# harmoniqs/DirectTrajOpt.jl

Hardware: AMD Instinct MI355X
Metric: knot-points/sec for eval_constraint_jacobian, 256-state×2000-knot bilinear (higher is better)
Workload: dtype f64; 1 GPU; configs[2]: 256-state bilinear, 4 drives, N=2000 knots per GPU (make_scaled_problem shape, Philox seed 42), callback=jacobian; state_dim=256, drives=4, knots_per_gpu=2000, knots_total=2000, parallelism=knot-range shards x1, outputs_finite=True, max_squarings=1, sweep_terms=25

## Files before the change

### directtrajopt.jl_amd/csrc/dto_engine.cpp

```cpp
#include "dto_handle.h"
#include "dto_rollout_plan.h"

#include <chrono>
#include <cmath>
#include <cstddef>
#include <cstdlib>
#include <cstring>
#include <initializer_list>
#include <limits>
#include <map>

using namespace dto;

thread_local std::string dto::g_create_error;

dto_handle::~dto_handle() {
    if (structure_only) return;
    (void)hipSetDevice(device);
    comm.reset();
    for (auto& r : prof) {
        (void)hipEventDestroy(r.a);
        (void)hipEventDestroy(r.b);
    }
    for (auto& e : ev_pool) (void)hipEventDestroy(e);
    for (void* p : owned) (void)hipFree(p);
    if (mailbox) (void)hipHostFree(mailbox);
    if (stream) (void)hipStreamDestroy(stream);
    if (stream2) (void)hipStreamDestroy(stream2);
    if (stream_rb) (void)hipStreamDestroy(stream_rb);
    if (ev_rb) (void)hipEventDestroy(ev_rb);
    if (ev_fork) (void)hipEventDestroy(ev_fork);
    if (ev_zero) (void)hipEventDestroy(ev_zero);
    if (ev_join) (void)hipEventDestroy(ev_join);
    if (ev_stats) (void)hipEventDestroy(ev_stats);
    if (ev_chain) (void)hipEventDestroy(ev_chain);
    if (ev_done) (void)hipEventDestroy(ev_done);
    if (h_stats) (void)hipHostFree(h_stats);
}

namespace {

struct ProfScope {
    dto_handle* h;
    hipStream_t st;
    bool on;
    ProfRec r{};
    ProfScope(dto_handle* h_, hipStream_t st_, int cat, double flops) : h(h_), st(st_), on(h_->profiling) {
        if (!on) return;
        r.cat = cat;
        r.flops = flops;
        auto take = [&](hipEvent_t& e) {
            if (h->ev_pool.empty()) (void)hipEventCreate(&e);
            else { e = h->ev_pool.back(); h->ev_pool.pop_back(); }
        };
        take(r.a);
        take(r.b);
        (void)hipEventRecord(r.a, st);
    }
    ~ProfScope() {
        if (!on) return;
        (void)hipEventRecord(r.b, st);
        h->prof.push_back(r);
    }
};
enum { CAT_BGEMM = 0, CAT_SWEEP = 1, CAT_OTHER = 2, CAT_BGEMM_HORNER = 3, CAT_BGEMM_SQUARE = 4, CAT_SWEEP_ADJOINT = 5,
       CAT_ZERO = 6, CAT_BUILD_A = 7, CAT_ASSEMBLY = 8, CAT_BASIS_MULTI = 9, CAT_CHAIN64 = 10, CAT_HESS_PRODUCT = 11, CAT_SHARE = 12, CAT_TDB_MFMA = 13, CAT_JAC_PRODUCT = 14, CAT_TDB_KRON = 15, CAT_TDB_PRODUCT = 16, CAT_ROLLOUT = 17, CAT_ROLLOUT_TREE = 18, CAT_ROLLOUT_DESCENT = 19, CAT_DYNSOLVE_TREE = 20, CAT_DYNSOLVE_SCAN = 21 };
inline bool is_rollout_cat(int cat) { return cat >= CAT_ROLLOUT && cat <= CAT_ROLLOUT_DESCENT; }
inline bool is_dynsolve_cat(int cat) { return cat == CAT_DYNSOLVE_TREE || cat == CAT_DYNSOLVE_SCAN; }
inline void count_sweep_form(dto_handle* h, int form) {
    if (h->profiling) ++h->sweep_forms[form];
}

}


namespace dto {

ShardExtents shard_extents(const dto_handle* h, int64_t k_lo, int64_t k_hi) {
    const int64_t kn_lo = k_lo - 1, n_knots = k_hi - k_lo + 1;
    const int64_t c_lo = kn_lo * h->z, c_hi = (kn_lo + n_knots) * h->z;
    const bool last = k_hi == h->N;
    ShardExtents e;
    e.grad_lo = c_lo;
    e.grad_len = c_hi - c_lo + (last ? h->gd : 0);
    e.jac_lo = h->colptr[c_lo];
    e.jac_len = h->colptr[last ? h->n_vars : c_hi] - e.jac_lo;
    e.hess_lo = hess_block_start(slab_dims(h), kn_lo);
    e.hess_len = hess_block_start(slab_dims(h), kn_lo + n_knots) - e.hess_lo + (last ? (int64_t)h->tail_rows.size() : 0);
    return e;
}

std::vector<std::pair<int64_t, int64_t>> shard_row_segments(const dto_handle* h, int64_t k_lo, int64_t k_hi) {
    const int64_t kn_lo = k_lo - 1, n_knots = k_hi - k_lo + 1;
    const int64_t n_int = std::max<int64_t>(0, std::min<int64_t>(k_hi, h->K) - k_lo + 1);
    std::vector<std::pair<int64_t, int64_t>> seg;
    for (size_t i = 0; i < h->integ_kind.size(); ++i)
        if (n_int > 0) seg.emplace_back(h->integ_row_off[i] + kn_lo * h->integ_dim[i], n_int * h->integ_dim[i]);
    for (auto& c : h->con) {
        int64_t prev = -2;
        for (int64_t i = 0; i < c.n_times_total; ++i) {
            const int64_t kn = c.times0[i];
            if (kn >= h->N ? k_hi != h->N : (kn < kn_lo || kn >= kn_lo + n_knots)) continue;
            if (!seg.empty() && prev == i - 1 && seg.back().first + seg.back().second == c.row_off + i * c.g_dim)
                seg.back().second += c.g_dim;
            else
                seg.emplace_back(c.row_off + i * c.g_dim, c.g_dim);
            prev = i;
        }
    }
    return seg;
}

}

namespace {



struct Bounds {
    double beta, b1;
};
Bounds read_bounds(const dto_handle* h) { return Bounds{h->mailbox->bounds[0], h->mailbox->bounds[1]}; }

void enqueue_bounds(dto_handle* h, BilHost& b, const double* dZ, hipStream_t st) {
    HIP_CHECK(hipMemsetAsync(h->d_bounds, 0, 2 * sizeof(double), st));
    launch_norm_bounds(st, h->P, b.k, dZ, b.d_g1, b.d_n2, reinterpret_cast<unsigned long long*>(h->d_bounds));
    HIP_CHECK(hipMemcpyAsync(h->mailbox->bounds, h->d_bounds, 2 * sizeof(double), hipMemcpyDeviceToHost, st));
}
Bounds get_bounds(dto_handle* h, BilHost& b, const double* dZ, hipStream_t st) {
    enqueue_bounds(h, b, dZ, st);
    HIP_CHECK(hipStreamSynchronize(st));
    return read_bounds(h);
}
// ... 109 lines not shown
                ps.r.flops += flops_step;
                if (a.store) {
                    ws.Z[0] = w.Zt + (size_t)t * tstride;
                    ws.Z[1] = w.Zt + (size_t)(t + 1) * tstride;
                    const bool split = ty.T == 1 && (int64_t)(t + b.k.m + 4) <= (int64_t)w.dcap * (1 + b.k.m);
                    launch_sweep_step(st, b.k, ws, ty, a.transposed, t, 0, split ? 1 : 0);
                } else {
                    launch_sweep_step(st, b.k, w, ty, a.transposed, t, buf);
                }
            }
            if (t >= tc) launch_sweep_check(st, w, ty.T, t, 1.1e-16);
            buf ^= 1;
            launched = t + 1;
            if (t >= 3 && (t % 4) == 3 && t + 1 < plan.d_ub) {
                int32_t* hs = h->mailbox->sweep_stats;
                if (pending) {
                    HIP_CHECK(hipEventSynchronize(h->ev_stats));
                    if (hs[slot ^ 1] == 0) break;
                }
                HIP_CHECK(hipMemcpyAsync(hs + slot, w.stats, sizeof(int32_t), hipMemcpyDeviceToHost, st));
                HIP_CHECK(hipEventRecord(h->ev_stats, st));
                pending = true;
                slot ^= 1;
            }
        }
    }
    return launched;
}

struct ChainChunks {
    int cap = 0;
    std::function<void(int64_t, int)> done;
};

struct ChainCall {
    ChainChunks chunks;
    std::function<void()> in_bubble;
    std::function<void(double)> after_last_enqueue;
    bool nothing_waits = false;
};

void run_chain(dto_handle* h, BilHost& b, const double* dZ, double* vals, hipStream_t st, const ChainCall& call) {
    const int npad = b.k.npad;
    const int64_t nint = h->P.n_int;
    double d2max = 0.0;
    if (nint <= 0) return;
    int cap = h->chain_chunk > 0 ? std::min(h->chain_chunk, b.chain_cap) : b.chain_cap;
    if (call.chunks.cap > 0 && !h->deterministic) cap = std::min(cap, call.chunks.cap);
    const int s_ub = 60;
    if (chain64_applies(h, b)) {
        ChainWork& w = b.chain;
        HIP_CHECK(hipMemsetAsync(w.smax, 0, 8 * sizeof(int32_t), st));
        HIP_CHECK(hipMemsetAsync(b.d_hump, 0, 8 * sizeof(unsigned long long), st));
        const int want_form = h->expm_form == 2 || h->expm_form == 3 ? h->expm_form : 0;
        {
            ProfScope ps(h, st, CAT_CHAIN64, 6.0 * 2.0 * 64.0 * 64.0 * 64.0 * (double)nint);
            HIP_CHECK(launch_chain64(st, h->P, b.k, dZ, vals, w.norms, w.smax, w.d2max, w.s, s_ub, want_form, h->n_cu));
        }
        if (call.nothing_waits) {
            HIP_CHECK(hipMemcpyAsync(&h->mailbox->deferred_smax, w.smax, sizeof(int32_t), hipMemcpyDeviceToHost, st));
            h->smax_pending = true;
            h->last_form = 0;
            if (call.in_bubble) call.in_bubble();
            if (call.chunks.done) call.chunks.done(0, (int)nint);
            if (call.after_last_enqueue) call.after_last_enqueue(0.0);
            return;
        }
        launch_hump(st, h->P, b.k, dZ, b.d_g1, h->P.kn_lo, (int)nint, w.norms, b.d_hump);
        const ChainReadback& rb = h->mailbox->chain;
        HIP_CHECK(hipMemcpyAsync(&h->mailbox->chain, w.smax, sizeof(ChainReadback), hipMemcpyDeviceToHost, st));
        HIP_CHECK(hipMemcpyAsync(h->mailbox->hump, b.d_hump, 8 * sizeof(unsigned long long), hipMemcpyDeviceToHost, st));
        HIP_CHECK(hipEventRecord(h->ev_chain, st));
        if (call.in_bubble) call.in_bubble();
        HIP_CHECK(hipEventSynchronize(h->ev_chain));
        h->last_form = 0;
        h->last_smax = rb.s_max2;
        read_hump(h, b);
        d2max = rb.d2max;
        if (call.chunks.done) call.chunks.done(0, (int)nint);
        if (call.after_last_enqueue) call.after_last_enqueue(d2max);
        return;
    }
    const double gemm_flops = 2.0 * npad * (double)npad * npad;
    h->last_smax = 0;
    const int64_t nchunk = (nint + cap - 1) / cap;
    const int per = (int)std::min<int64_t>(cap, (((nint + nchunk - 1) / nchunk) + 7) / 8 * 8);
    for (int64_t c0 = 0; c0 < nint; c0 += per) {
        const int nb = (int)std::min<int64_t>(per, nint - c0);
        const int64_t int0 = h->P.kn_lo + c0;
        ChainWork& w = b.chain;
        const int nbpad = ((nb + 127) / 128) * 128;
        if (b.use_basis) {
            launch_fill(st, w.norms, (int64_t)nb * 4, INFINITY);
            double* outs[3] = {w.W[1], w.W[2], w.W[3]};
            const size_t cs_set = (size_t)cap * npad * (npad / 64);
            double* css[3] = {w.colsum, w.colsum + cs_set, w.colsum + 2 * cs_set};
            {
                ProfScope ps(h, st, CAT_BUILD_A, 8.0 * npad * (double)npad * nb);
                launch_build_A(st, h->P, b.k, dZ, int0, nb, w.W[0]);
            }
            launch_basis_coef_multi(st, h->P, b.k, 3, b.basis, dZ, int0, nb, nbpad);
            {
                const double cols = b.basis[0].cntpad + b.basis[1].cntpad + b.basis[2].cntpad;
                ProfScope ps(h, st, CAT_BASIS_MULTI, 2.0 * npad * (double)npad * cols * nb);
                launch_basis_gemm_multi(st, npad, nb, nbpad, 3, b.basis, outs, css);
            }
            launch_norm_from_colsum_multi(st, npad, nb, 3, css, w.norms);
        } else {
            {
                ProfScope ps(h, st, CAT_BUILD_A, 8.0 * npad * (double)npad * nb);
                launch_build_A(st, h->P, b.k, dZ, int0, nb, w.W[0]);
            }
            { ProfScope ps(h, st, CAT_BGEMM, gemm_flops * nb); launch_bgemm_plain(st, npad, nb, w.W[0], w.W[0], w.W[1]); }
            { ProfScope ps(h, st, CAT_BGEMM, gemm_flops * nb); launch_bgemm_plain(st, npad, nb, w.W[0], w.W[1], w.W[2]); }
            { ProfScope ps(h, st, CAT_BGEMM, gemm_flops * nb); launch_bgemm_plain(st, npad, nb, w.W[1], w.W[1], w.W[3]); }
            launch_norm1(st, npad, nb, w);
        }
        HIP_CHECK(hipMemsetAsync(w.smax, 0, 8 * sizeof(int32_t), st));
        launch_expm_params(st, nb, s_ub, w);
        if (c0 == 0) HIP_CHECK(hipMemsetAsync(b.d_hump, 0, 8 * sizeof(unsigned long long), st));
        launch_hump(st, h->P, b.k, dZ, b.d_g1, int0, nb, w.norms, b.d_hump);
        launch_expm_coef(st, nb, w, h->expm_form == 2 || h->expm_form == 3 ? h->expm_form : 0);
        const ChainReadback& rb = h->mailbox->chain;
        HIP_CHECK(hipEventRecord(h->ev_rb, st));
        HIP_CHECK(hipStreamWaitEvent(h->stream_rb, h->ev_rb, 0));
        HIP_CHECK(hipMemcpyAsync(&h->mailbox->chain, w.smax, sizeof(ChainReadback), hipMemcpyDeviceToHost, h->stream_rb));
        HIP_CHECK(hipMemcpyAsync(h->mailbox->hump, b.d_hump, 8 * sizeof(unsigned long long), hipMemcpyDeviceToHost, h->stream_rb));
        HIP_CHECK(hipEventRecord(h->ev_chain, h->stream_rb));
        if (b.use_basis) {
            launch_basis_coef(st, h->P, b.k, b.basis_all, dZ, int0, nb, nbpad, w.coef);
            ProfScope ps(h, st, CAT_OTHER, 2.0 * npad * (double)npad * b.basis_all.cntpad * nb);
            launch_basis_gemm(st, npad, nb, nbpad, b.basis_all, w.W[5], nullptr);
        } else {
            launch_poly_h3(st, npad, nb, w);
        }
        if (c0 == 0 && call.in_bubble) call.in_bubble();
        HIP_CHECK(hipEventSynchronize(h->ev_chain));
        const int form = rb.form;
        if (form != 2 && form != 3) throw HipError{"propagator chain: the evaluation form did not come back from the device"};
        h->last_form = form;
        { ProfScope ps(h, st, CAT_BGEMM_HORNER, gemm_flops * nb); launch_bgemm_poly(st, npad, nb, w, 3, 5, 4, COEF_PA, 6, COEF_PB); }
        const SlabDest slab{h->P, b.k, int0, vals};
        if (form == 2) {
            ProfScope ps(h, st, CAT_BGEMM_HORNER, gemm_flops * nb);
            launch_bgemm_poly(st, npad, nb, w, 4, 6, 5, COEF_PC, -1, 0, false, &slab);
        } else {
            { ProfScope ps(h, st, CAT_BGEMM_HORNER, gemm_flops * nb); launch_bgemm_poly(st, npad, nb, w, 4, 6, 7, COEF_L, 8, COEF_R, true); }
            { ProfScope ps(h, st, CAT_BGEMM_HORNER, gemm_flops * nb); launch_bgemm_poly(st, npad, nb, w, 7, 8, 5, COEF_PC, -1, 0, false, &slab); }
        }
        const int s_max = form == 3 ? rb.s_max3 : rb.s_max2;
        const int s_sum = form == 3 ? rb.s_sum3 : rb.s_sum2;
        read_hump(h, b);
        const double dv = rb.d2max;
        d2max = (dv == dv) ? std::max(d2max, dv) : dv;
        const double sq_flops = s_max > 0 ? gemm_flops * (double)s_sum / s_max : 0.0;
        h->last_smax = std::max(h->last_smax, s_max);
        int src = 5;
        for (int it = 0; it < s_max; ++it) {
            ProfScope ps(h, st, CAT_BGEMM_SQUARE, sq_flops);
            launch_bgemm_square(st, npad, nb, w, src, src == 4 ? 5 : 4, it, h->P, b.k, int0, vals);
            src = src == 4 ? 5 : 4;
        }
        if (call.chunks.done) call.chunks.done(c0, nb);
    }
    if (call.after_last_enqueue) call.after_last_enqueue(d2max);
}

double exact_d2(dto_handle* h, BilHost& b, const double* dZ, hipStream_t st, bool higher = false) {
    const int npad = b.k.npad;
    const int64_t nint = h->P.n_int;
    double d2max = 0.0;
    for (int64_t c0 = 0; c0 < nint; c0 += b.chain_cap) {
        const int nb = (int)std::min<int64_t>(b.chain_cap, nint - c0);
        const int64_t int0 = h->P.kn_lo + c0;
        ChainWork& w = b.chain;
        HIP_CHECK(hipMemsetAsync(w.smax, 0, 8 * sizeof(int32_t), st));
        launch_fill(st, w.norms, (int64_t)nb * 4, INFINITY);
        if (c0 == 0) HIP_CHECK(hipMemsetAsync(b.d_hump, 0, 8 * sizeof(unsigned long long), st));
        if (b.use_basis) {
            const int nbpad = ((nb + 127) / 128) * 128;
            const int nr = higher ? 3 : 1;
            for (int r = 0; r < nr; ++r) {
                double* cs = w.colsum + (size_t)r * b.chain_cap * npad * (npad / 64);
                launch_basis_coef(st, h->P, b.k, b.basis[r], dZ, int0, nb, nbpad, nullptr);
                launch_basis_gemm(st, npad, nb, nbpad, b.basis[r], nullptr, cs);
                launch_norm_from_colsum(st, npad, nb, cs, w.norms, 1 + r, higher ? nullptr : w.d2max);
            }
            if (higher) launch_beta_from_norms(st, nb, w);
        } else {
            launch_build_A(st, h->P, b.k, dZ, int0, nb, w.W[0]);
            launch_bgemm_plain(st, npad, nb, w.W[0], w.W[0], w.W[1]);
            launch_norm1_one(st, npad, nb, w, 1);
        }
        launch_hump(st, h->P, b.k, dZ, b.d_g1, int0, nb, w.norms, b.d_hump);
        HIP_CHECK(hipMemcpyAsync(&h->mailbox->chain, w.smax, offsetof(ChainReadback, s_max3), hipMemcpyDeviceToHost, st));
        HIP_CHECK(hipMemcpyAsync(h->mailbox->hump, b.d_hump, 8 * sizeof(unsigned long long), hipMemcpyDeviceToHost, st));
        HIP_CHECK(hipStreamSynchronize(st));
        const double dv = h->mailbox->chain.d2max;
        d2max = (dv == dv) ? std::max(d2max, dv) : dv;
    }
    read_hump(h, b);
    return d2max;
}

void read_hump(dto_handle* h, BilHost& b) {
    const unsigned long long* hp = h->mailbox->hump;
    b.hump_valid = true;
    for (int q = 0; q < 4; ++q) {
        double v;
        memcpy(&v, &hp[q], sizeof(double));
        b.hump_logH[q] = v;
        b.hump_kend[q] = (int)hp[4 + q];
        if (!(v == v)) b.hump_valid = false;
    }
}
// ... 1804 lines not shown
    if (std::string(name) == "expm_form") {
        if (value != 0 && value != 2 && value != 3) return fail(h, "dto_set_option: expm_form takes 0 (by cost), 2 or 3");
        h->expm_form = (int)value;
        return 0;
    }
    return fail(h, std::string("dto_set_option: unknown option ") + name);
}

int dto_profile_enable(dto_handle* h, int32_t on) {
    if (!h) return 1;
    if (on && !h->structure_only && h->ev_pool.size() < 1024) {
        (void)hipSetDevice(h->device);
        while (h->ev_pool.size() < 1024) {
            hipEvent_t e;
            if (hipEventCreate(&e) != hipSuccess) break;
            h->ev_pool.push_back(e);
        }
    }
    h->profiling = on != 0;
    return 0;
}
int dto_profile_reset(dto_handle* h) {
    if (!h) return 1;
    for (auto& r : h->prof) { h->ev_pool.push_back(r.a); h->ev_pool.push_back(r.b); }
    h->prof.clear();
    for (auto& c : h->sweep_forms) c = 0;
    return 0;
}
int dto_profile_get(dto_handle* h, const char* name, double* ms, int64_t* launches, double* flops) {
    return guarded(h, [&] {
        int cat = -1;
        bool any_gemm = false, any_basis = false, any_rollout = false, any_dynsolve = false;
        if (!strcmp(name, "bgemm")) any_gemm = true;
        else if (!strcmp(name, "bgemm_horner")) cat = CAT_BGEMM_HORNER;
        else if (!strcmp(name, "bgemm_square")) cat = CAT_BGEMM_SQUARE;
        else if (!strcmp(name, "bgemm_plain")) cat = CAT_BGEMM;
        else if (!strcmp(name, "chain64")) cat = CAT_CHAIN64;
        else if (!strcmp(name, "basis")) any_basis = true;
        else if (!strcmp(name, "basis_k")) cat = CAT_OTHER;
        else if (!strcmp(name, "basis_multi")) cat = CAT_BASIS_MULTI;
        else if (!strcmp(name, "zero_fill")) cat = CAT_ZERO;
        else if (!strcmp(name, "build_A")) cat = CAT_BUILD_A;
        else if (!strcmp(name, "assembly")) cat = CAT_ASSEMBLY;
        else if (!strcmp(name, "expmv")) cat = CAT_SWEEP;
        else if (!strcmp(name, "expmv_adjoint")) cat = CAT_SWEEP_ADJOINT;
        else if (!strcmp(name, "hess_product")) cat = CAT_HESS_PRODUCT;
        else if (!strcmp(name, "share")) cat = CAT_SHARE;
        else if (!strcmp(name, "tdb_mfma")) cat = CAT_TDB_MFMA;
        else if (!strcmp(name, "tdb_kron")) cat = CAT_TDB_KRON;
        else if (!strcmp(name, "jac_product")) cat = CAT_JAC_PRODUCT;
        else if (!strcmp(name, "tdb_product")) cat = CAT_TDB_PRODUCT;
        else if (!strcmp(name, "rollout")) any_rollout = true;
        else if (!strcmp(name, "rollout_gather")) cat = CAT_ROLLOUT;
        else if (!strcmp(name, "rollout_tree")) cat = CAT_ROLLOUT_TREE;
        else if (!strcmp(name, "rollout_descent")) cat = CAT_ROLLOUT_DESCENT;
        else if (!strcmp(name, "dynsolve")) any_dynsolve = true;
        else if (!strcmp(name, "dynsolve_tree")) cat = CAT_DYNSOLVE_TREE;
        else if (!strcmp(name, "dynsolve_scan")) cat = CAT_DYNSOLVE_SCAN;
        else if (!strcmp(name, "hess_product_setup")) {
            if (ms) *ms = h->hp_setup_ms;
            if (launches) *launches = 0;
            if (flops) *flops = h->hp_bytes;
            return;
        }
        else if (!strncmp(name, "sweep_", 6)) {
            static const char* const forms[5] = {"sweep_gs", "sweep_fused", "sweep_s64", "sweep_cluster", "sweep_step"};
            int f = 0;
            while (f < 5 && strcmp(name, forms[f])) ++f;
            if (f == 5) throw HipError{"dto_profile_get: unknown name"};
            if (ms) *ms = 0.0;
            if (launches) *launches = h->sweep_forms[f];
            if (flops) *flops = 0.0;
            return;
        }
        else if (strcmp(name, "all")) throw HipError{"dto_profile_get: unknown name"};
        double tot = 0, fl = 0;
        int64_t n = 0;
        for (auto& r : h->prof) {
            if (any_gemm && r.cat != CAT_BGEMM && r.cat != CAT_BGEMM_HORNER && r.cat != CAT_BGEMM_SQUARE && r.cat != CAT_CHAIN64) continue;
            if (any_basis && r.cat != CAT_OTHER && r.cat != CAT_BASIS_MULTI) continue;
            if (!any_gemm && !any_basis && cat >= 0 && r.cat != cat) continue;
            if (is_rollout_cat(r.cat) ? !(any_rollout || r.cat == cat) : any_rollout) continue;
            if (is_dynsolve_cat(r.cat) ? !(any_dynsolve || r.cat == cat) : any_dynsolve) continue;
            HIP_CHECK(hipEventSynchronize(r.b));
            float t = 0;
            HIP_CHECK(hipEventElapsedTime(&t, r.a, r.b));
            tot += t; ++n;
            if (cat == CAT_SHARE || r.cat != CAT_SHARE) fl += r.flops;
        }
        if (ms) *ms = tot;
        if (launches) *launches = n;
        if (flops) *flops = fl;
    });
}
int dto_last_stats(const dto_handle* h, int32_t* max_squarings, int32_t* expmv_terms) {
    if (!h) return 1;
    dto_handle* hm = const_cast<dto_handle*>(h);
    int rc = guarded(hm, [&] { HIP_CHECK(hipDeviceSynchronize()); }, G_BLOCKING);
    if (max_squarings) *max_squarings = h->last_smax;
    if (expmv_terms) *expmv_terms = h->last_terms;
    return rc;
}

}
```

### directtrajopt.jl_amd/csrc/dto_handle.h

```cpp
#pragma once

#include "../../include/dto_engine.h"

#include <hip/hip_runtime.h>

#include <algorithm>
#include <cstdio>
#include <functional>
#include <memory>
#include <string>
#include <type_traits>
#include <utility>
#include <vector>

#include "dto_comm.h"
#include "dto_hostxfer.h"
#include "dto_kernels.h"
#include "dto_sweep_cache.h"

namespace dto {

extern thread_local std::string g_create_error;

struct HipError {
// ... 44 lines not shown
    int chain_cap = 0;
    unsigned long long* d_hump = nullptr;
    double hump_logH[4] = {0, 0, 0, 0};
    int hump_kend[4] = {0, 0, 0, 0};
    bool hump_valid = false;
    SweepCache cache;
    SweepWork cluster_work[2];
    SweepWork gs_work[2];
    bool small = false;
    double* d_Gs = nullptr;
    bool use_basis = false;
    BasisSet basis[3]{};
    BasisSet basis_all{};
    bool pairing = false;
    double* EP = nullptr;
    double* Upair = nullptr;
    double* d_Btab = nullptr;
    int kb = 0, kr = 1;
    bool kron = false;
    KKron kk{};
    double* d_kron_scratch = nullptr;
    size_t kron_stride = 0;
    int share_leader = -1, share_size = 1, list_pos = 0;
    bool share_active = false;
    std::vector<int> share_followers;
    bool follows() const { return share_active && share_followers.empty(); }
};

struct ConHost {
    KCon k{};
    int equality = 0;
    int64_t n_times_total = 0;
    int64_t row_off = 0;
    std::vector<int64_t> times0;
    std::vector<int32_t> comps;
    int g_dim = 1;
    bool external = false;
    bool global = false;
    int ext_slot = -1;
    std::vector<double> jac0;
    std::vector<double> hess0;
    std::vector<double> M;
    KExtTerm xk{};
};

struct ExtObjHost {
    double weight = 1.0;
    bool global = false;
    std::vector<int32_t> comps, gcomps;
    std::vector<int64_t> times0;
    KExtTerm k{};
    int ext_slot = -1;
};

struct ExtSlot {
    dto_external_values v{nullptr, nullptr, nullptr};
    size_t len[3] = {0, 0, 0};
    double* d[3] = {nullptr, nullptr, nullptr};
};

struct TdbHost {
    KTdb k{};
    KExtInt place{};
    double *d_vals = nullptr, *d_jac = nullptr, *d_hess = nullptr, *d_scratch = nullptr;
    size_t stride = 0;
    double* d_jtv = nullptr;
    bool mfma = false;
    double *d_Bp = nullptr, *d_BpT = nullptr;
    int resident = 0;
    int kb = 0, kr = 1;
    bool kron = false;
    KKron kk{};
    int share_leader = -1, share_size = 1, share_cap = 1, list_pos = 0;
    bool share_active = false;
    std::vector<int> share_members;
    double* d_share_scratch = nullptr;
    size_t share_stride = 0;
};

struct ProfRec {
    hipEvent_t a, b;
    int cat;
    double flops;
};

struct ChainReadback {
    int32_t s_max2, s_sum2;
    double d2max;
    int32_t s_max3, s_sum3;
    int32_t form;
    int32_t pad;
};
static_assert(sizeof(ChainReadback) == 32 && std::is_standard_layout<ChainReadback>::value, "ChainReadback mirrors eight int32 of ChainWork::smax");

struct PinnedMailbox {
    double bounds[2];
    ChainReadback chain;
    int32_t sweep_stats[2];
    unsigned long long hump[8];
    int32_t same_flag;
    int32_t hp_flag;
    int32_t dyn_flag;
    int32_t deferred_smax;
};
}

struct dto_handle {
    std::string err;
    int device = 0;
    bool structure_only = false;
    int64_t N = 0, K = 0;
    int z = 0, gd = 0, dt_idx = 0, D = 0;
    int eval_hessian = 1;
    int64_t n_vars = 0, n_cons = 0, n_dyn = 0, jac_nnz = 0, hess_nnz = 0;
    int64_t k_lo = 1, k_hi = 1;
    dto::KProb P{};
    std::vector<int64_t> colptr;
    std::vector<int64_t> con_cols, con_rows;
    std::vector<dto::BilHost> bil;
    std::vector<dto::KDer> der;
    std::vector<int> integ_kind, integ_index;
    std::vector<int> integ_dim;
    std::vector<int64_t> integ_row_off;
    std::vector<dto::ConHost> con;
    std::vector<dto::KObj> obj;
    struct ObjInfo {
        int kind, comp_off, comp_dim;
        std::vector<int32_t> comps;
        std::vector<int64_t> times;
        std::vector<int64_t> layer_start;
    };
    std::vector<ObjInfo> obj_info;
    std::unique_ptr<dto::HostXfer> xfer;
    dto::XferPlan jac_plan, hess_plan;
    bool plans_built = false;
    bool raw_plans_built = false;
    double* bound[2] = {nullptr, nullptr};
    bool primed[2] = {false, false};
    int64_t* d_bind_start[2] = {nullptr, nullptr};
    int64_t* d_bind_len[2] = {nullptr, nullptr};
    int64_t n_bind_runs[2] = {0, 0};
    bool bind_ready[2] = {false, false};
    int host_xfer = 1;
    int xfer_check = 0;
    std::vector<dto::ExtObjHost> ext_obj;
    std::vector<dto::KExtInt> ext_int;
    std::vector<dto::TdbHost> tdb;
    std::vector<dto::ExtSlot> ext;
    int n_ext_int = 0, n_ext_con = 0, n_ext_obj = 0;
    std::vector<int64_t> tail_colptr, tail_rows;
    int64_t hess_block_nnz = 0;
    std::vector<std::pair<int64_t, int64_t>> row_segments;
    int64_t cons_len = 0;
    dto_shard_info info{};

    int64_t* d_colptr = nullptr;
    double* d_Z = nullptr;
    double* d_mu = nullptr;
    double* d_out = nullptr;
    size_t d_out_cap = 0;
    double* d_partial = nullptr;
    double* d_f = nullptr;
    double* d_bounds = nullptr;
    int32_t* d_plan = nullptr;
    double* d_jac_scratch = nullptr;
    double* d_w = nullptr;
// ... 104 lines not shown
```

### directtrajopt.jl_amd/csrc/dto_kernels.h

```cpp
#pragma once
#include <hip/hip_runtime.h>
#include <stdint.h>

#include <cstdlib>

#include "dto_slab_layout.h"
#include "dto_sweep_plan.h"

namespace dto {

constexpr int TAYLOR_M = 16;
constexpr double THETA_16 = 0.78028743;
constexpr int COEF_STRIDE = 32;
constexpr int COEF_PC = 0, COEF_PA = 5, COEF_PB = 10, COEF_K = 15;
constexpr double EXPM2_K[5] = {0.0021247619694343247, 0.00021337327385069214, 1.9238573871783716e-05, 1.748961261071247e-06, 2.1862015763390587e-07};
constexpr double EXPM2_A[5] = {0.15657629060017847, 0.11131927651852432, 0.04459108138499527, 0.00629379053080652, -0.00037523326035530425};
constexpr double EXPM2_B[5] = {6.392946474783064, 1.8714151425525498, 0.2847453199197648, 0.035205562271892026, 0.0005680709246076226};
constexpr double EXPM2_C[5] = {-0.000983845027019532, -0.004677417588383601, -0.03797734224052902, 0.005772376398520401, 0.0016659351281941514};
constexpr double THETA_3P = 2.8188;
constexpr int COEF_L = 20, COEF_R = 26;
constexpr double EXPM3_K[5] = {0.00010379876595047617, 6.073095185901804e-06, 3.1522969877676845e-07, -5.57963065580417e-09, 1.6549758371825144e-09};
constexpr double EXPM3_A[5] = {0.06925346208946212, 0.1399878337730723, 0.008815043145043342, -1.5454750321185654e-05, 0.0};
constexpr double EXPM3_B[5] = {7.864692916335445, 1.1432871789700823, 0.08599260924787294, 0.006001949142362251, 0.000114009585419753};
constexpr double EXPM3_C[5] = {1.4279329585415197, -0.648965244154349, -0.10937992097592901, -0.0031202517331481694, 0.0};
// ... 275 lines not shown
    const double* R;
    const double* baseline;
    const int64_t* times;
    int64_t n_times;
    const int32_t* comps;
    int32_t n_comps, pad1;
    const double* params;
    const double* Qs;
    const int32_t* last;
};
void launch_objective(hipStream_t st, const KProb& P, const KObj& O, const double* dZ, double* partial, double* f);
void launch_gradient(hipStream_t st, const KProb& P, const KObj& O, const double* dZ, double* grad);
void launch_hess_objective(hipStream_t st, const KProb& P, const KObj& O, const double* dZ, double sigma, double* H);
void launch_hess_derivative(hipStream_t st, const KProb& P, const KDer& Dv, const double* dmu, double* H);
void launch_hess_bilinear(hipStream_t st, const KProb& P, const KBil& B, const SweepBuf& fw, const SweepBuf& ad,
                          const double* dmu, double* H, int with_uu);

constexpr int SHARE_MAX_FOLLOWERS = 15;
struct KShare {
    int32_t n, nf;
    int32_t x_off[1 + SHARE_MAX_FOLLOWERS];
    int32_t pre[1 + SHARE_MAX_FOLLOWERS];
};
void launch_share_E(hipStream_t st, const KProb& P, const KShare& S, int64_t int0, int nb, double* vals);

struct KRollout {
    int32_t n, npad, x_off, pre;
    int32_t n_cols, col_pad;
    int32_t L;
    int64_t K;
};
void launch_rollout_leaves(hipStream_t st, const KProb& P, const KRollout& R, const double* vals, double* tree);
void launch_rollout_start(hipStream_t st, const KRollout& R, const double* dZ, const double* X0, double* S);
void launch_rollout_descend(hipStream_t st, const KRollout& R, int l, int64_t only, const double* tree, double* S);
void launch_rollout_compact(hipStream_t st, const KRollout& R, int64_t k0, int64_t nk, const double* S, double* X);

void launch_dynsolve_load(hipStream_t st, const KRollout& R, int adjoint, const double* B, double* off, double* S);
void launch_dynsolve_up(hipStream_t st, const KRollout& R, int adjoint, int l, const double* tree, double* off);
void launch_dynsolve_descend(hipStream_t st, const KRollout& R, int adjoint, int l, int64_t only, const double* tree, double* off, double* S);

void launch_fill(hipStream_t st, double* p, int64_t n, double v);
void launch_zero_runs(hipStream_t st, const int64_t* start, const int64_t* len, int64_t n_runs, double* dst);

size_t small_lds_bytes(int n, int m, int T_fw, int T_ad);
hipError_t small_prepare(size_t lds_bytes);
hipError_t launch_small(hipStream_t st, const KProb& P, const KBil& B, const double* Gs, const SweepTypes& ty_fw,
                        const SweepTypes& ty_ad, const double* dZ, const double* dmu, double* cons, double* jac, double* hess,
                        int mode);

struct KIntegTable {
    int32_t n;
    int32_t d[8];
    int64_t off[8];
};
void launch_jac_spmv(hipStream_t st, const KProb& P, const KIntegTable& T, const int64_t* conbase, const int64_t* con_rows,
                     const double* vals, const double* w, double* y, int transpose, int64_t global_cols = 0);
void launch_jac_rowgather(hipStream_t st, const KProb& P, const KIntegTable& T, int64_t n_con_rows, const int64_t* rptr, const int64_t* rcol,
                          const int64_t* rpos, int64_t n_dyn, const double* vals, const double* w, double* y);
void launch_add(hipStream_t st, double* dst, const double* src, int64_t n);
void launch_bits_equal(hipStream_t st, const double* a, const double* b, int64_t n, int32_t* flag);

struct KHessProduct {
    const int64_t* start;
    const int32_t* len;
    const int32_t* col;
    const double* val;
    const int32_t* rows;
    int64_t row0[4], blk0[4];
    int32_t cls_g[3];
    int32_t n_cls;
};
void launch_hess_gather(hipStream_t st, const double* slab, const int64_t* pos, int64_t n, double* val);
void launch_hess_spmv(hipStream_t st, const KHessProduct& p, const double* v, double* y);

struct BasisSet {
    int32_t r, cnt, cntpad;
    const double* S;
    const int32_t* idx;
    double* coef;
};
void launch_basis_coef(hipStream_t st, const KProb& P, const KBil& B, const BasisSet& bs, const double* dZ,
                       int64_t int0, int nb, int nbpad, const double* taylor);
void launch_jac_zero(hipStream_t st, const KProb& P, const KBil& B, double* vals);
void launch_basis_gemm(hipStream_t st, int npad, int nb, int nbpad, const BasisSet& bs, double* out, double* colsum);
void launch_basis_gemm_multi(hipStream_t st, int npad, int nb, int nbpad, int nsets, const BasisSet* bs, double* const* out,
                             double* const* colsum);
void launch_basis_coef_multi(hipStream_t st, const KProb& P, const KBil& B, int nsets, const BasisSet* bs, const double* dZ,
                             int64_t int0, int nb, int nbpad);
void launch_norm_from_colsum_multi(hipStream_t st, int npad, int nb, int nsets, double* const* colsum, double* norms);
void launch_beta_from_norms(hipStream_t st, int nb, const ChainWork& w);
void launch_hump(hipStream_t st, const KProb& P, const KBil& B, const double* dZ, const double* g1, int64_t int0, int nb,
                 const double* norms, unsigned long long* out);
void launch_norm_from_colsum(hipStream_t st, int npad, int nb, const double* colsum, double* norms, int which,
                             unsigned long long* d2max = nullptr);
void launch_norm_bounds(hipStream_t st, const KProb& P, const KBil& B, const double* dZ, const double* g1,
                        const double* n2, unsigned long long* out2);

}
```

### directtrajopt.jl_amd/csrc/dto_kernels.hip

```cpp
#include "dto_bgemm_dispatch.h"
#include "dto_gemm.hip.h"
#include "dto_gemm_ring.hip.h"
#include "dto_kernels.h"
#include "dto_hostxfer.h"

#include <cstdlib>

namespace dto {

__device__ __forceinline__ unsigned long long dbits(double v) { return (unsigned long long)__double_as_longlong(fabs(v)); }
__device__ __forceinline__ double bits_to_d(unsigned long long b) { return __longlong_as_double((long long)b); }

__device__ __forceinline__ void hess_add(const KProb& P, double* H, int64_t kn, int a, int b, double v);

static inline dim3 blk(const KProb& P, int threads) { return dim3(P.debug_bad_launch ? 4096 : threads); }

__device__ __forceinline__ double wave_sum(double v) {
#pragma unroll
    for (int o = 32; o > 0; o >>= 1) v += __shfl_xor(v, o, 64);
    return v;
}
__device__ __forceinline__ double wave_max(double v) {
#pragma unroll
    for (int o = 32; o > 0; o >>= 1) v = fmax(v, __shfl_xor(v, o, 64));
// ... 57 lines not shown
    double* p = dst + start[r];
    const int64_t n = len[r];
    for (int64_t i = threadIdx.x & 63; i < n; i += 64) p[i] = 0.0;
}
void launch_zero_runs(hipStream_t st, const int64_t* start, const int64_t* len, int64_t n_runs, double* dst) {
    if (n_runs <= 0) return;
    hipLaunchKernelGGL(k_zero_runs, dim3((unsigned)((n_runs + 3) / 4)), dim3(256), 0, st, start, len, n_runs, dst);
}

void launch_add(hipStream_t st, double* dst, const double* src, int64_t n) {
    if (n <= 0) return;
    int grid = (int)((n + 255) / 256 < 4096 ? (n + 255) / 256 : 4096);
    hipLaunchKernelGGL(k_add, dim3(grid), dim3(256), 0, st, dst, src, n);
}

__global__ void k_basis_coef(KProb P, KBil B, BasisSet bs, const double* __restrict__ Z, int64_t int0, int nb,
                             const double* __restrict__ taylor) {
    const int b = blockIdx.x;
    double* c = bs.coef + (int64_t)b * bs.cntpad;
    if (b >= nb) {
        for (int a = threadIdx.x; a < bs.cntpad; a += blockDim.x) c[a] = 0.0;
        return;
    }
    const double* zk = Z + (int0 + b) * P.z;
    const double dt = zk[P.dt_idx];
    for (int a = threadIdx.x; a < bs.cntpad; a += blockDim.x) {
        double v = 0.0;
        if (a < bs.cnt) {
            v = 1.0;
            int deg = 0;
            for (int i = 0; i < bs.r; ++i) {
                const int g = bs.idx[a * bs.r + i];
                if (g < 0) continue;
                ++deg;
                v *= dt;
                if (g > 0) v *= zk[B.u_off + g - 1];
            }
            if (taylor) v *= taylor[(int64_t)b * COEF_STRIDE + COEF_K + deg];
        }
        c[a] = v;
    }
}
void launch_basis_coef(hipStream_t st, const KProb& P, const KBil& B, const BasisSet& bs, const double* dZ,
                       int64_t int0, int nb, int nbpad, const double* taylor) {
    hipLaunchKernelGGL(k_basis_coef, dim3(nbpad), dim3(128), 0, st, P, B, bs, dZ, int0, nb, taylor);
}

template <class Cfg>
__device__ __forceinline__ void basis_epilogue(const GemmAccS<Cfg>& acc, int npad, int nb, int rt, int ct, double* __restrict__ out,
                                               double* __restrict__ colsum) {
    constexpr int TM = Cfg::TM, TN = Cfg::TN;
    static_assert(Cfg::WTM == 64, "column sums assume 64-row wave tiles");
    const int64_t nn = (int64_t)npad * npad;
    const int wave_row0 = rt * TM + ((threadIdx.x >> 6) / Cfg::WC) * Cfg::WTM;
    GemmCoordP<Cfg> co;
    const int row0 = rt * TM + co.row_base, col0 = ct * TN + co.col_base;
#pragma unroll
    for (int tj = 0; tj < Cfg::NT; ++tj)
#pragma unroll
        for (int r = 0; r < 4; ++r) {
            const int col = col0 + 16 * tj + 4 * r;
            double asum = 0.0;
#pragma unroll
            for (int p = 0; p < Cfg::MT / 2; ++p) {
                const d2 v = {acc.v[2 * p][tj][r], acc.v[2 * p + 1][tj][r]};
                if (out && col < nb) __builtin_nontemporal_store(v, reinterpret_cast<d2*>(&out[(int64_t)col * nn + row0 + 32 * p]));
                asum += fabs(v.x) + fabs(v.y);
            }
            if (colsum) {
#pragma unroll
                for (int o = 8; o > 0; o >>= 1) asum += __shfl_xor(asum, o, 64);
                if ((threadIdx.x & 15) == 0 && col < nb) colsum[((int64_t)col * npad + wave_row0 / npad) * (npad / 64) + (wave_row0 % npad) / 64] = asum;
            }
        }
}
template <class Cfg>
__device__ __forceinline__ void basis_accumulate(GemmAccS<Cfg>& acc, const BasisSet& bs, int64_t nn, int rt, int ct, double* smem) {
    const double* A = bs.S + (int64_t)rt * Cfg::TM;
    const double* B = bs.coef + (int64_t)ct * Cfg::TN * bs.cntpad;
    gemm_accumulate_p<Cfg>(acc, A, (int)nn, B, bs.cntpad, bs.cntpad, smem);
}

template <class Cfg>
__global__ void __launch_bounds__(Cfg::THREADS, 2) k_basis_gemm(int npad, int nb, BasisSet bs, double* __restrict__ out,
                                                                double* __restrict__ colsum) {
    __shared__ __attribute__((aligned(1024))) double smem[Cfg::SMEM_DOUBLES];
    const int64_t nn = (int64_t)npad * npad;
    const int row_tiles = (int)(nn / Cfg::TM);
    const int rt = blockIdx.x % row_tiles, ct = blockIdx.x / row_tiles;
    GemmAccS<Cfg> acc;
    acc.zero();
    basis_accumulate<Cfg>(acc, bs, nn, rt, ct, smem);
    basis_epilogue<Cfg>(acc, npad, nb, rt, ct, out, colsum);
}
__global__ void k_norm_from_colsum(int npad, int nb, const double* __restrict__ colsum, double* __restrict__ norms, int which,
                                   unsigned long long* d2max) {
    const int b = blockIdx.x;
    double m = 0.0;
    const int nch = npad / 64;
    auto colsum_of = [&](int c) {
        double v = 0.0;
        for (int q = 0; q < nch; ++q) v += colsum[((int64_t)b * npad + c) * nch + q];
        return v;
    };
    for (int c = threadIdx.x; c < npad; c += 64) m = fmax(m, colsum_of(c));
    m = wave_max(m);
    double bad = 0.0;
    for (int c = threadIdx.x; c < npad; c += 64) { const double v = colsum_of(c); if (!(v == v)) bad = 1.0; }
    bad = wave_max(bad);
    if (threadIdx.x == 0) {
        const double v = bad > 0.0 ? __longlong_as_double(0x7ff8000000000000ll) : m;
        norms[b * 4 + which] = v;
        if (d2max) atomicMax(d2max, dbits(sqrt(v)));
    }
}
void launch_norm_from_colsum(hipStream_t st, int npad, int nb, const double* colsum, double* norms, int which,
                             unsigned long long* d2max) {
    hipLaunchKernelGGL(k_norm_from_colsum, dim3(nb), dim3(64), 0, st, npad, nb, colsum, norms, which, d2max);
}
struct BasisMulti {
    int nsets;
    BasisSet bs[4];
    double* out[4];
    double* colsum[4];
};
template <class Cfg>
__global__ void __launch_bounds__(Cfg::THREADS, 2) k_basis_gemm_multi(int npad, int nb, BasisMulti M) {
    __shared__ __attribute__((aligned(1024))) double smem[Cfg::SMEM_DOUBLES];
    const int which = blockIdx.x % M.nsets, tile = blockIdx.x / M.nsets;
    BasisSet bs = M.bs[0];
    double* out = M.out[0];
    double* colsum = M.colsum[0];
#pragma unroll
    for (int q = 1; q < 4; ++q)
        if (q == which) { bs = M.bs[q]; out = M.out[q]; colsum = M.colsum[q]; }
    const int64_t nn = (int64_t)npad * npad;
    const int row_tiles = (int)(nn / Cfg::TM);
    const int rt = tile % row_tiles, ct = tile / row_tiles;
    GemmAccS<Cfg> acc;
    acc.zero();
    basis_accumulate<Cfg>(acc, bs, nn, rt, ct, smem);
    basis_epilogue<Cfg>(acc, npad, nb, rt, ct, out, colsum);
}
void launch_basis_gemm_multi(hipStream_t st, int npad, int nb, int nbpad, int nsets, const BasisSet* bs, double* const* out,
                             double* const* colsum) {
    const int64_t nn = (int64_t)npad * npad;
    BasisMulti M{};
    M.nsets = nsets;
    for (int q = 0; q < nsets; ++q) { M.bs[q] = bs[q]; M.out[q] = out[q]; M.colsum[q] = colsum[q]; }
    const dim3 grid((unsigned)((nn / 128) * (nbpad / 128) * nsets));
    using C = GemmShapeP<128, 128, 2, 4>;
    hipLaunchKernelGGL((k_basis_gemm_multi<C>), grid, dim3(C::THREADS), 0, st, npad, nb, M);
}
__global__ void k_basis_coef_multi(KProb P, KBil B, BasisMulti M, const double* __restrict__ Z, int64_t int0, int nb) {
    const int b = blockIdx.x;
    BasisSet bs = M.bs[0];
#pragma unroll
    for (int q = 1; q < 4; ++q)
        if (q == (int)blockIdx.y) bs = M.bs[q];
    double* c = bs.coef + (int64_t)b * bs.cntpad;
    if (b >= nb) {
        for (int a = threadIdx.x; a < bs.cntpad; a += blockDim.x) c[a] = 0.0;
        return;
    }
    const double* zk = Z + (int0 + b) * P.z;
    const double dt = zk[P.dt_idx];
    for (int a = threadIdx.x; a < bs.cntpad; a += blockDim.x) {
        double v = 0.0;
        if (a < bs.cnt) {
            v = 1.0;
            for (int i = 0; i < bs.r; ++i) {
                const int g = bs.idx[a * bs.r + i];
                v *= dt;
                if (g > 0) v *= zk[B.u_off + g - 1];
            }
        }
        c[a] = v;
    }
}
void launch_basis_coef_multi(hipStream_t st, const KProb& P, const KBil& B, int nsets, const BasisSet* bs, const double* dZ,
                             int64_t int0, int nb, int nbpad) {
    BasisMulti M{};
    M.nsets = nsets;
    for (int q = 0; q < nsets; ++q) M.bs[q] = bs[q];
    hipLaunchKernelGGL(k_basis_coef_multi, dim3(nbpad, nsets), dim3(128), 0, st, P, B, M, dZ, int0, nb);
}
__global__ void k_norm_from_colsum_multi(int npad, int nb, BasisMulti M, double* __restrict__ norms) {
    const int b = blockIdx.x, which = blockIdx.y;
    const double* colsum = M.colsum[0];
#pragma unroll
    for (int q = 1; q < 3; ++q)
        if (q == which) colsum = M.colsum[q];
    double m = 0.0, bad = 0.0;
    const int nch = npad / 64;
    for (int c = threadIdx.x; c < npad; c += 64) {
        double v = 0.0;
        for (int q = 0; q < nch; ++q) v += colsum[((int64_t)b * npad + c) * nch + q];
        m = fmax(m, v);
        if (!(v == v)) bad = 1.0;
    }
    m = wave_max(m);
    bad = wave_max(bad);
    if (threadIdx.x == 0) norms[b * 4 + 1 + which] = bad > 0.0 ? __longlong_as_double(0x7ff8000000000000ll) : m;
}
void launch_norm_from_colsum_multi(hipStream_t st, int npad, int nb, int nsets, double* const* colsum, double* norms) {
    BasisMulti M{};
    M.nsets = nsets;
    for (int q = 0; q < nsets; ++q) M.colsum[q] = colsum[q];
    hipLaunchKernelGGL(k_norm_from_colsum_multi, dim3(nb, nsets), dim3(64), 0, st, npad, nb, M, norms);
}
void launch_basis_gemm(hipStream_t st, int npad, int nb, int nbpad, const BasisSet& bs, double* out, double* colsum) {
    const int64_t nn = (int64_t)npad * npad;
    const dim3 grid((unsigned)((nn / 128) * (nbpad / 128)));
    using C = GemmShapeP<128, 128, 2, 4>;
    hipLaunchKernelGGL((k_basis_gemm<C>), grid, dim3(C::THREADS), 0, st, npad, nb, bs, out, colsum);
}

template <int TRANSPOSE>
__global__ void __launch_bounds__(64) k_jac_spmv(KProb P, KIntegTable T, const int64_t* __restrict__ conbase,
                                                 const int64_t* __restrict__ con_rows, const double* __restrict__ vals,
                                                 const double* __restrict__ w, double* __restrict__ y) {
    const int64_t cl = blockIdx.x;
    const int64_t c = P.kn_lo * P.z + cl;
    const int64_t kn = c / P.z;
    const int has_prev = kn >= 1 && kn < P.N, has_own = kn < P.K;
    const int cnt = has_prev + has_own;
    const int64_t e0 = P.colptr[c], e1 = P.colptr[c + 1];
    const int64_t Lint = (int64_t)P.D * cnt;
    static_assert(TRANSPOSE == 1, "J w takes the row gather (launch_jac_rowgather): a column walk would meet other columns in y[row]");
    double acc = 0.0;
    for (int64_t e = e0 + threadIdx.x; e < e1; e += 64) {
        const int64_t el = e - e0;
        int64_t row;
        if (el < Lint) {
            int64_t rem = el;
            int i = 0;
            while (i < T.n - 1 && rem >= (int64_t)T.d[i] * cnt) { rem -= (int64_t)T.d[i] * cnt; ++i; }
            const int d = T.d[i];
            if (has_prev && rem < d) row = T.off[i] + (kn - 1) * d + rem;
            else row = T.off[i] + kn * d + (rem - (has_prev ? d : 0));
        } else {
            row = con_rows[conbase[c] + (el - Lint)];
        }
        const double v = vals[e - P.jac_lo];
        acc += v * w[row];
    }
    acc = wave_sum(acc);
    if (threadIdx.x == 0) y[c] = acc;
}
__global__ void __launch_bounds__(64) k_jac_rowgather_integ(KProb P, KIntegTable T, const double* __restrict__ vals,
                                                            const double* __restrict__ w, double* __restrict__ y) {
    const int64_t R = blockIdx.x;
    int i = 0, pre = 0;
    while (i < T.n - 1 && R >= T.off[i] + (int64_t)T.d[i] * P.K) { pre += T.d[i]; ++i; }
    const int d = T.d[i];
    const int64_t kn = (R - T.off[i]) / d;
    const int r = (int)((R - T.off[i]) % d);
    double acc = 0.0;
    for (int j = threadIdx.x; j < P.z; j += 64) {
        acc += vals[jac_pos(P, P.colptr, kn, j, pre, d, 1, r)] * w[kn * P.z + j];
        acc += vals[jac_pos(P, P.colptr, kn + 1, j, pre, d, 0, r)] * w[(kn + 1) * P.z + j];
    }
    acc = wave_sum(acc);
    if (threadIdx.x == 0) y[R] = acc;
}
__global__ void __launch_bounds__(64) k_jac_rowgather_con(const int64_t* __restrict__ rptr, const int64_t* __restrict__ rcol,
                                                          const int64_t* __restrict__ rpos, int64_t row0, const double* __restrict__ vals,
                                                          const double* __restrict__ w, double* __restrict__ y) {
    const int64_t r = blockIdx.x;
    double acc = 0.0;
    for (int64_t e = rptr[r] + threadIdx.x; e < rptr[r + 1]; e += 64) acc += vals[rpos[e]] * w[rcol[e]];
    acc = wave_sum(acc);
    if (threadIdx.x == 0) y[row0 + r] = acc;
}
void launch_jac_rowgather(hipStream_t st, const KProb& P, const KIntegTable& T, int64_t n_con_rows, const int64_t* rptr, const int64_t* rcol,
                          const int64_t* rpos, int64_t n_dyn, const double* vals, const double* w, double* y) {
    if (T.n > 0 && n_dyn > 0) hipLaunchKernelGGL(k_jac_rowgather_integ, dim3((unsigned)n_dyn), dim3(64), 0, st, P, T, vals, w, y);
    if (n_con_rows > 0) hipLaunchKernelGGL(k_jac_rowgather_con, dim3((unsigned)n_con_rows), dim3(64), 0, st, rptr, rcol, rpos, n_dyn, vals, w, y);
}
void launch_jac_spmv(hipStream_t st, const KProb& P, const KIntegTable& T, const int64_t* conbase, const int64_t* con_rows,
                     const double* vals, const double* w, double* y, int transpose, int64_t global_cols) {
    const int64_t ncols = P.n_knots * P.z + global_cols;
    if (ncols <= 0) return;
    (void)transpose;
    hipLaunchKernelGGL(k_jac_spmv<1>, dim3((unsigned)ncols), dim3(64), 0, st, P, T, conbase, con_rows, vals, w, y);
}

__global__ void __launch_bounds__(256) k_jac_zero(KProb P, KBil B, double* __restrict__ vals) {
    const int64_t kn = P.kn_lo + blockIdx.x;
    const int has_prev = kn >= 1, has_own = kn < P.K;
    const int cnt = has_prev + has_own;
    const bool skipE = has_own && (int64_t)blockIdx.x < P.n_int;
    const int64_t e_lo = (int64_t)B.pre * cnt + (has_prev ? B.n : 0);
    const int lane = threadIdx.x & 127, half = threadIdx.x >> 7;
    auto zero_range = [&](int64_t lo, int64_t hi) {
        if (hi <= lo) return;
        const int64_t a = lo + (int64_t)((reinterpret_cast<uintptr_t>(vals + lo) >> 3) & 1);
        if (lane == 0 && a > lo) vals[lo] = 0.0;
// ... 1734 lines not shown
```

Before: 189,400 knot-points/s.

## Fuse build_A into the basis GEMM epilogue on the basis chain path

On the basis path, the separate build_A kernel launch is skipped by default. A = sum_j u_j*dt*G_j is now computed inside the basis_all GEMM kernel after its epilogue, reusing the same tiles and the LDS for the coefficient table. This removes one kernel launch and lets the A build share the GEMM's grid, at the cost of more registers and work per GEMM block. W[0] is now produced later in the chain. That is fine only if nothing between the old and new points reads W[0]; basis_gemm_multi and coef seem to use basis coefficients rather than A.

```diff
diff --git a/directtrajopt.jl_amd/csrc/dto_engine.cpp b/directtrajopt.jl_amd/csrc/dto_engine.cpp
--- a/directtrajopt.jl_amd/csrc/dto_engine.cpp
+++ b/directtrajopt.jl_amd/csrc/dto_engine.cpp
@@ -45,10 +45,11 @@
     hipStream_t st;
     bool on;
     ProfRec r{};
-    ProfScope(dto_handle* h_, hipStream_t st_, int cat, double flops) : h(h_), st(st_), on(h_->profiling) {
+    ProfScope(dto_handle* h_, hipStream_t st_, int cat, double flops, bool shadow = false) : h(h_), st(st_), on(h_->profiling) {
         if (!on) return;
         r.cat = cat;
         r.flops = flops;
+        r.shadow = shadow;
         auto take = [&](hipEvent_t& e) {
             if (h->ev_pool.empty()) (void)hipEventCreate(&e);
             else { e = h->ev_pool.back(); h->ev_pool.pop_back(); }
@@ -324,6 +325,7 @@
         return;
     }
     const double gemm_flops = 2.0 * npad * (double)npad * npad;
+    static const int a_from_k = tune_int("DTO_CHAIN_A_FROM_K", 1);
     h->last_smax = 0;
     const int64_t nchunk = (nint + cap - 1) / cap;
     const int per = (int)std::min<int64_t>(cap, (((nint + nchunk - 1) / nchunk) + 7) / 8 * 8);
@@ -337,7 +339,7 @@
             double* outs[3] = {w.W[1], w.W[2], w.W[3]};
             const size_t cs_set = (size_t)cap * npad * (npad / 64);
             double* css[3] = {w.colsum, w.colsum + cs_set, w.colsum + 2 * cs_set};
-            {
+            if (!a_from_k) {
                 ProfScope ps(h, st, CAT_BUILD_A, 8.0 * npad * (double)npad * nb);
                 launch_build_A(st, h->P, b.k, dZ, int0, nb, w.W[0]);
             }
@@ -372,7 +374,13 @@
         if (b.use_basis) {
             launch_basis_coef(st, h->P, b.k, b.basis_all, dZ, int0, nb, nbpad, w.coef);
             ProfScope ps(h, st, CAT_OTHER, 2.0 * npad * (double)npad * b.basis_all.cntpad * nb);
-            launch_basis_gemm(st, npad, nb, nbpad, b.basis_all, w.W[5], nullptr);
+            if (a_from_k) {
+                ProfScope pa(h, st, CAT_BUILD_A, 8.0 * npad * (double)npad * nb, true);
+                const BasisBuildA ba = basis_build_A_args(h->P, b.k, dZ, int0, w.W[0]);
+                launch_basis_gemm(st, npad, nb, nbpad, b.basis_all, w.W[5], nullptr, &ba);
+            } else {
+                launch_basis_gemm(st, npad, nb, nbpad, b.basis_all, w.W[5], nullptr);
+            }
         } else {
             launch_poly_h3(st, npad, nb, w);
         }
@@ -2343,6 +2351,7 @@
             if (!any_gemm && !any_basis && cat >= 0 && r.cat != cat) continue;
             if (is_rollout_cat(r.cat) ? !(any_rollout || r.cat == cat) : any_rollout) continue;
             if (is_dynsolve_cat(r.cat) ? !(any_dynsolve || r.cat == cat) : any_dynsolve) continue;
+            if (r.shadow && r.cat != cat) continue;
             HIP_CHECK(hipEventSynchronize(r.b));
             float t = 0;
             HIP_CHECK(hipEventElapsedTime(&t, r.a, r.b));
diff --git a/directtrajopt.jl_amd/csrc/dto_handle.h b/directtrajopt.jl_amd/csrc/dto_handle.h
--- a/directtrajopt.jl_amd/csrc/dto_handle.h
+++ b/directtrajopt.jl_amd/csrc/dto_handle.h
@@ -150,6 +150,7 @@
     hipEvent_t a, b;
     int cat;
     double flops;
+    bool shadow = false;
 };
 
 struct ChainReadback {
diff --git a/directtrajopt.jl_amd/csrc/dto_kernels.h b/directtrajopt.jl_amd/csrc/dto_kernels.h
--- a/directtrajopt.jl_amd/csrc/dto_kernels.h
+++ b/directtrajopt.jl_amd/csrc/dto_kernels.h
@@ -381,7 +381,18 @@
 void launch_basis_coef(hipStream_t st, const KProb& P, const KBil& B, const BasisSet& bs, const double* dZ,
                        int64_t int0, int nb, int nbpad, const double* taylor);
 void launch_jac_zero(hipStream_t st, const KProb& P, const KBil& B, double* vals);
-void launch_basis_gemm(hipStream_t st, int npad, int nb, int nbpad, const BasisSet& bs, double* out, double* colsum);
+struct BasisBuildA {
+    const double* G;
+    const double* Z;
+    double* A;
+    int64_t int0;
+    int32_t z, dt_idx, u_off, m;
+};
+inline BasisBuildA basis_build_A_args(const KProb& P, const KBil& B, const double* dZ, int64_t int0, double* A) {
+    return BasisBuildA{B.G, dZ, A, int0, P.z, P.dt_idx, B.u_off, B.m};
+}
+void launch_basis_gemm(hipStream_t st, int npad, int nb, int nbpad, const BasisSet& bs, double* out, double* colsum,
+                       const BasisBuildA* with_A = nullptr);
 void launch_basis_gemm_multi(hipStream_t st, int npad, int nb, int nbpad, int nsets, const BasisSet* bs, double* const* out,
                              double* const* colsum);
 void launch_basis_coef_multi(hipStream_t st, const KProb& P, const KBil& B, int nsets, const BasisSet* bs, const double* dZ,
diff --git a/directtrajopt.jl_amd/csrc/dto_kernels.hip b/directtrajopt.jl_amd/csrc/dto_kernels.hip
--- a/directtrajopt.jl_amd/csrc/dto_kernels.hip
+++ b/directtrajopt.jl_amd/csrc/dto_kernels.hip
@@ -163,16 +163,88 @@
 }
 
 template <class Cfg>
+struct BasisBuildATile {
+    static constexpr int NP = Cfg::MT / 2, GJ = 5;
+    d2 g[GJ][NP];
+    int64_t nn, row0;
+    int col0, col_base;
+    __device__ __forceinline__ void load_group(const BasisBuildA& ba, int j0) {
+#pragma unroll
+        for (int jj = 0; jj < GJ; ++jj)
+#pragma unroll
+            for (int p = 0; p < NP; ++p)
+                g[jj][p] = j0 + jj <= ba.m ? *reinterpret_cast<const d2*>(ba.G + (int64_t)(j0 + jj) * nn + row0 + 32 * p) : d2{0.0, 0.0};
+    }
+    __device__ __forceinline__ void fetch(const BasisBuildA& ba, int npad, int nb, int rt, int ct, double* cu) {
+        GemmCoordP<Cfg> co;
+        nn = (int64_t)npad * npad;
+        row0 = (int64_t)rt * Cfg::TM + co.row_base;
+        col0 = ct * Cfg::TN + co.col_base;
+        col_base = co.col_base;
+        load_group(ba, 0);
+        for (int e = threadIdx.x; e < (ba.m + 1) * Cfg::TN; e += Cfg::THREADS) {
+            const int j = e / Cfg::TN, col = ct * Cfg::TN + e % Cfg::TN;
+            double v = 0.0;
+            if (col < nb) {
+                const double* zk = ba.Z + (ba.int0 + col) * ba.z;
+                v = zk[ba.dt_idx];
+                if (j > 0) v = v * zk[ba.u_off + j - 1];
+            }
+            cu[e] = v;
+        }
+        __syncthreads();
+    }
+    __device__ __forceinline__ void store(const BasisBuildA& ba, int nb, const double* cu) {
+#pragma unroll 1
+        for (int tj = 0; tj < Cfg::NT; ++tj) {
+            d2 av[4][NP];
+#pragma unroll
+            for (int r = 0; r < 4; ++r)
+#pragma unroll
+                for (int p = 0; p < NP; ++p) av[r][p] = d2{0.0, 0.0};
+            for (int j0 = 0; j0 <= ba.m; j0 += GJ) {
+                if (j0 > 0) load_group(ba, j0);
+#pragma unroll
+                for (int jj = 0; jj < GJ; ++jj)
+                    if (j0 + jj <= ba.m) {
+#pragma unroll
+                        for (int r = 0; r < 4; ++r) {
+                            const double ub = cu[(j0 + jj) * Cfg::TN + col_base + 16 * tj + 4 * r];
+#pragma unroll
+                            for (int p = 0; p < NP; ++p) {
+                                av[r][p].x += ub * g[jj][p].x;
+                                av[r][p].y += ub * g[jj][p].y;
+                            }
+                        }
+                    }
+            }
+            if (ba.m >= GJ && tj + 1 < Cfg::NT) load_group(ba, 0);
+#pragma unroll
+            for (int r = 0; r < 4; ++r) {
+                const int col = col0 + 16 * tj + 4 * r;
+#pragma unroll
+                for (int p = 0; p < NP; ++p)
+                    if (col < nb) __builtin_nontemporal_store(av[r][p], reinterpret_cast<d2*>(&ba.A[(int64_t)col * nn + row0 + 32 * p]));
+            }
+        }
+    }
+};
+
+template <class Cfg, bool WITH_A = false>
 __global__ void __launch_bounds__(Cfg::THREADS, 2) k_basis_gemm(int npad, int nb, BasisSet bs, double* __restrict__ out,
-                                                                double* __restrict__ colsum) {
+                                                                double* __restrict__ colsum, BasisBuildA ba) {
     __shared__ __attribute__((aligned(1024))) double smem[Cfg::SMEM_DOUBLES];
+    static_assert((MAX_DRIVES + 1) * Cfg::TN <= Cfg::SMEM_DOUBLES, "the coefficient table of BasisBuildATile fits the panels' LDS");
     const int64_t nn = (int64_t)npad * npad;
     const int row_tiles = (int)(nn / Cfg::TM);
     const int rt = blockIdx.x % row_tiles, ct = blockIdx.x / row_tiles;
     GemmAccS<Cfg> acc;
     acc.zero();
     basis_accumulate<Cfg>(acc, bs, nn, rt, ct, smem);
+    BasisBuildATile<Cfg> at;
+    if constexpr (WITH_A) at.fetch(ba, npad, nb, rt, ct, smem);
     basis_epilogue<Cfg>(acc, npad, nb, rt, ct, out, colsum);
+    if constexpr (WITH_A) at.store(ba, nb, smem);
 }
 __global__ void k_norm_from_colsum(int npad, int nb, const double* __restrict__ colsum, double* __restrict__ norms, int which,
                                    unsigned long long* d2max) {
@@ -290,11 +362,13 @@
     for (int q = 0; q < nsets; ++q) M.colsum[q] = colsum[q];
     hipLaunchKernelGGL(k_norm_from_colsum_multi, dim3(nb, nsets), dim3(64), 0, st, npad, nb, M, norms);
 }
-void launch_basis_gemm(hipStream_t st, int npad, int nb, int nbpad, const BasisSet& bs, double* out, double* colsum) {
+void launch_basis_gemm(hipStream_t st, int npad, int nb, int nbpad, const BasisSet& bs, double* out, double* colsum,
+                       const BasisBuildA* with_A) {
     const int64_t nn = (int64_t)npad * npad;
     const dim3 grid((unsigned)((nn / 128) * (nbpad / 128)));
     using C = GemmShapeP<128, 128, 2, 4>;
-    hipLaunchKernelGGL((k_basis_gemm<C>), grid, dim3(C::THREADS), 0, st, npad, nb, bs, out, colsum);
+    if (with_A) hipLaunchKernelGGL((k_basis_gemm<C, true>), grid, dim3(C::THREADS), 0, st, npad, nb, bs, out, colsum, *with_A);
+    else hipLaunchKernelGGL((k_basis_gemm<C, false>), grid, dim3(C::THREADS), 0, st, npad, nb, bs, out, colsum, BasisBuildA{});
 }
 
 template <int TRANSPOSE>
```

After: 192,000 knot-points/s (median of 6 runs). +1.4%, better.
